# mit-han-lab/distrifuser

Hardware: NVIDIA H100
Metric: SDXL 50-step latency (ms/image) (lower is better)
Workload: dtype f16

## Files before the change

### distrifuser_b200/csrc/linear.cu

```cuda
#include <math.h>
#include <string.h>

#include "tc_ptx.cuh"

using namespace df;
using namespace df::tc;

namespace {

constexpr int BM = 128;
constexpr int BK = 64;
constexpr int NTHREADS = 288;
constexpr int NCONSUMER_WARPS = 8;
constexpr uint32_t A_BYTES = BM * BK * 2;

template <int BN> struct Stages { static constexpr int value = BN == 256 ? 4 : 5; };

template <int BN>
struct __align__(1024) SmemT {
  __half a[Stages<BN>::value][BM * BK];
  __half b[Stages<BN>::value][BN * BK];
  uint64_t full[Stages<BN>::value], empty[Stages<BN>::value];
};

enum { EPI_PLAIN = 0, EPI_GEGLU = 1 };

struct LinearArgs {
  const __half* bias;
  const __half* residual;
  __half* out;
  int64_t M;
  int N, K;
  int64_t ldr, ldo;
  int tiles_m, tiles_n;
  int publish;
  int pub_col0, pub_cols;
  int idx;
  uint32_t peer_mask;
  uint64_t tensor_off, slot_bytes;
  df_comm_t comm;
};

__device__ __forceinline__ float gelu_erf(float x) {
  const float z = fabsf(x) * 0.70710678118654752f;
  const float t = __fdividef(1.f, fmaf(0.3275911f, z, 1.f));
  float p = fmaf(1.061405429f, t, -1.453152027f);
  p = fmaf(p, t, 1.421413741f);
  p = fmaf(p, t, -0.284496736f);
  p = fmaf(p, t, 0.254829592f);
  const float e = p * t * __expf(-z * z);
  const float phi = x >= 0.f ? 1.f - 0.5f * e : 0.5f * e;
  return x * phi;
}

__device__ __forceinline__ float2 ld_h2f(const __half* p) { return __half22float2(*reinterpret_cast<const __half2*>(p)); }

template <int BN>
__device__ __forceinline__ void wgmma_tile(float* acc, uint64_t a_desc, uint64_t b_desc, uint32_t accumulate) {
  if constexpr (BN == 256) wgmma_ss_n256(acc, a_desc, b_desc, accumulate);
  else wgmma_ss_n160(acc, a_desc, b_desc, accumulate);
}

template <int EPI, int BN>
__global__ void __launch_bounds__(NTHREADS, 1)
linear_kernel(const __grid_constant__ CUtensorMap tm_a, const __grid_constant__ CUtensorMap tm_w, LinearArgs p) {
  static_assert(BN % 32 == 0 && BN <= 256 && (BN * BK * 2) % 1024 == 0, "tile shape");
  constexpr int STAGES = Stages<BN>::value;
  constexpr uint32_t B_BYTES = BN * BK * 2;
  using Smem = SmemT<BN>;
  extern __shared__ __align__(1024) uint8_t smem_raw[];
  Smem& sm = *reinterpret_cast<Smem*>(smem_raw);
  if ((smem_u32(smem_raw) & 1023u) != 0) __trap();
  const int warp = threadIdx.x >> 5, lane = threadIdx.x & 31;
  const int ntiles = p.tiles_m * p.tiles_n;
  const int kblocks = p.K / BK;

  if (threadIdx.x == 0) {
    for (int s = 0; s < STAGES; ++s) { mbar_init(&sm.full[s], 1); mbar_init(&sm.empty[s], NCONSUMER_WARPS); }
    asm volatile("fence.mbarrier_init.release.cluster;" ::: "memory");
  }
  __syncthreads();
  pdl_wait();

  if (warp == NCONSUMER_WARPS) {
    if (lane == 0) {
      prefetch_tmap(&tm_a);
      prefetch_tmap(&tm_w);
      uint32_t stage = 0, phase = 0;
      for (int tile = blockIdx.x; tile < ntiles; tile += gridDim.x) {
        const int tm = tile % p.tiles_m, tn = tile / p.tiles_m;
        for (int kb = 0; kb < kblocks; ++kb) {
          mbar_wait(&sm.empty[stage], phase ^ 1u);
          mbar_expect_tx(&sm.full[stage], A_BYTES + B_BYTES);
          tma_load_2d(sm.a[stage], &tm_a, &sm.full[stage], kb * BK, tm * BM);
          tma_load_2d(sm.b[stage], &tm_w, &sm.full[stage], kb * BK, tn * BN);
          if (++stage == STAGES) { stage = 0; phase ^= 1u; }
        }
      }
    }
  } else {
    const int wg = warp >> 2;
    const int c4 = lane & 3;
    const int rloc = wg * 64 + (warp & 3) * 16 + (lane >> 2);
    uint32_t pub_epoch = 0;
    if (p.publish) pub_epoch = p.comm.clock[0];
    uint32_t stage = 0, phase = 0;
    float acc[BN / 2];
    for (int tile = blockIdx.x; tile < ntiles; tile += gridDim.x) {
      const int tm = tile % p.tiles_m, tn = tile / p.tiles_m;
      fence_regs<BN / 2>(acc);
      uint32_t prev = 0;
      for (int kb = 0; kb < kblocks; ++kb) {
        mbar_wait(&sm.full[stage], phase);
        const uint32_t a_addr = smem_u32(sm.a[stage]) + wg * 64 * 128, b_addr = smem_u32(sm.b[stage]);
        wgmma_fence();
#pragma unroll
        for (int kk = 0; kk < BK / 16; ++kk)
          wgmma_tile<BN>(acc, smem_desc(a_addr + kk * 32, 16, 1024), smem_desc(b_addr + kk * 32, 16, 1024), (kb | kk) > 0);
        wgmma_commit();
        wgmma_wait<1>();
        if (kb > 0 && lane == 0) mbar_arrive(&sm.empty[prev]);
        prev = stage;
        if (++stage == STAGES) { stage = 0; phase ^= 1u; }
      }
      wgmma_wait<0>();
      fence_regs<BN / 2>(acc);
      if (lane == 0) mbar_arrive(&sm.empty[prev]);
#pragma unroll
      for (int h = 0; h < 2; ++h) {
        const int64_t grow = (int64_t)tm * BM + rloc + 8 * h;
        if (grow >= p.M) continue;
        if (EPI == EPI_GEGLU) {
          __half* dst = p.out + grow * p.ldo + tn * (BN / 2);
#pragma unroll
          for (int i = 0; i < BN / 16; ++i) {
            const int c = 8 * i + 2 * c4;
            float2 bh = make_float2(0.f, 0.f), bg = make_float2(0.f, 0.f);
            if (p.bias) { bh = ld_h2f(p.bias + tn * BN + c); bg = ld_h2f(p.bias + tn * BN + BN / 2 + c); }
            const float* hv = acc + 4 * i + 2 * h;
            const float* gv = acc + 4 * (i + BN / 16) + 2 * h;
            const float2 hf = __half22float2(__floats2half2_rn(hv[0] + bh.x, hv[1] + bh.y));
            const float2 gf = __half22float2(__floats2half2_rn(gv[0] + bg.x, gv[1] + bg.y));
            *reinterpret_cast<__half2*>(dst + c) = __floats2half2_rn(hf.x * gelu_erf(gf.x), hf.y * gelu_erf(gf.y));
          }
        } else {
          const int col0 = tn * BN;
          __half* dst = p.out + grow * p.ldo + col0;
          const __half* res = p.residual ? p.residual + grow * p.ldr + col0 : nullptr;
#pragma unroll
          for (int i = 0; i < BN / 8; ++i) {
            const int c = 8 * i + 2 * c4;
            const int col = col0 + c;
            if (col >= p.N) continue;
            float2 f = make_float2(acc[4 * i + 2 * h], acc[4 * i + 2 * h + 1]);
            if (p.bias) { const float2 bb = ld_h2f(p.bias + col); f.x += bb.x; f.y += bb.y; }
            __half2 o = __floats2half2_rn(f.x, f.y);
            if (res) o = __hadd2(o, *reinterpret_cast<const __half2*>(res + c));
            *reinterpret_cast<__half2*>(dst + c) = o;
            if (p.publish && col >= p.pub_col0) {
              const uint64_t off = slot_offset(p.comm, pub_epoch, p.tensor_off, p.slot_bytes, p.comm.rank) +
                                   ((uint64_t)grow * p.pub_cols + (col - p.pub_col0)) * 2;
              for (int q = 0; q < p.comm.world; ++q)
                if (p.peer_mask >> q & 1) *reinterpret_cast<__half2*>((char*)p.comm.base[q] + off) = o;
            }
          }
        }
      }
    }
  }
  if (p.publish) signal_when_last(p.comm, &p.comm.tickets[p.idx], gridDim.x, p.idx, p.peer_mask, p.comm.clock[0]);
}

int make_map2d(CUtensorMap* m, const void* base, int64_t rows, int K, int64_t pitch, int box_rows) {
  EncodeTiledFn enc = tensor_map_encoder();
  DF_REQUIRE(enc != nullptr, "cuTensorMapEncodeTiled is not available from this driver");
  cuuint64_t dims[2] = {(cuuint64_t)K, (cuuint64_t)rows};
  cuuint64_t strides[1] = {(cuuint64_t)pitch * 2};
  cuuint32_t box[2] = {BK, (cuuint32_t)box_rows};
  cuuint32_t estr[2] = {1, 1};
  CUresult r = enc(m, CU_TENSOR_MAP_DATA_TYPE_FLOAT16, 2, const_cast<void*>(base), dims, strides, box, estr,
                   CU_TENSOR_MAP_INTERLEAVE_NONE, CU_TENSOR_MAP_SWIZZLE_128B, CU_TENSOR_MAP_L2_PROMOTION_L2_256B,
                   CU_TENSOR_MAP_FLOAT_OOB_FILL_NONE);
  DF_REQUIRE(r == CUDA_SUCCESS, "cuTensorMapEncodeTiled failed (%d): base=%p rows=%lld K=%d pitch=%lld", (int)r, base,
             (long long)rows, K, (long long)pitch);
  return 0;
}

template <int EPI, int BN>
int launch_linear(const CUtensorMap& ta, const CUtensorMap& tw, const LinearArgs& args, int ctas, cudaStream_t st) {
  static bool attr_set = false;
  if (!attr_set) {
    DF_CHECK_CUDA(cudaFuncSetAttribute(linear_kernel<EPI, BN>, cudaFuncAttributeMaxDynamicSharedMemorySize, (int)sizeof(SmemT<BN>)));
    attr_set = true;
  }
  DF_CHECK_CUDA(launch_pdl(PDL_GEMM, linear_kernel<EPI, BN>, dim3(ctas), dim3(NTHREADS), sizeof(SmemT<BN>), st, ta, tw, args));
  return 0;
}

double tile_cost(int64_t M, int N, int bn, int ctas_avail) {
  const long long tm = (M + BM - 1) / BM, tn = (N + bn - 1) / bn, tiles = tm * tn;
  const long long rounds = (tiles + ctas_avail - 1) / ctas_avail;
  return (double)rounds * (bn + 64);
}

}

namespace {
int pick_bn(int64_t M, int N, int epilogue, int cap) {
  const bool ok160 = epilogue == EPI_PLAIN || N % 160 == 0, ok256 = epilogue == EPI_PLAIN || N % 256 == 0;
  if (!ok256) return ok160 ? 160 : 0;
  if (ok160 && tile_cost(M, N, 160, cap) < 0.97 * tile_cost(M, N, 256, cap)) return 160;
  return 256;
}
}

extern "C" int df_linear_supported(int64_t M, int N, int K, int epilogue) {
  if (M < 1 || N < 8 || N % 8 != 0 || K < BK || K % BK != 0) return 0;
  if (epilogue == EPI_GEGLU && pick_bn(M, N, epilogue, sm_count()) == 0) return 0;
  return 1;
}

extern "C" int df_linear_geglu_block(int64_t M, int N, int K) {
  (void)K;
  const int bn = pick_bn(M, N, EPI_GEGLU, sm_count());
  return bn / 2;
}

extern "C" int df_linear_fwd(df_comm_t comm, const void* a, const void* w, const void* bias, const void* residual, void* out,
                             int64_t M, int N, int K, int64_t lda, int64_t ldw, int64_t ldr, int64_t ldo, int epilogue,
                             int geglu_block, int publish, int pub_col0, int idx, uint32_t peer_mask, uint64_t tensor_off,
                             uint64_t slot_bytes, int max_ctas, void* stream) {
  DF_REQUIRE(epilogue == EPI_PLAIN || epilogue == EPI_GEGLU, "df_linear_fwd: unknown epilogue %d", epilogue);
  DF_REQUIRE(df_linear_supported(M, N, K, epilogue), "df_linear_fwd: unsupported shape M=%lld N=%d K=%d (N %% 8, K %% 64%s)",
             (long long)M, N, K, epilogue == EPI_GEGLU ? ", GEGLU: N % 256" : "");
  DF_REQUIRE(((uintptr_t)a % 16) == 0 && ((uintptr_t)w % 16) == 0 && ((uintptr_t)out % 16) == 0 && ((uintptr_t)bias % 16) == 0 &&
                 ((uintptr_t)residual % 16) == 0 && lda % 8 == 0 && ldw % 8 == 0 && ldo % 8 == 0 && ldr % 8 == 0,
             "df_linear_fwd: operands must be 16-byte aligned with pitches multiple of 8");
  DF_REQUIRE(!(publish && epilogue != EPI_PLAIN), "df_linear_fwd: publication is a plain-epilogue feature");
  LinearArgs args;
  memset(&args, 0, sizeof(args));
  args.bias = (const __half*)bias; args.residual = (const __half*)residual; args.out = (__half*)out;
  args.M = M; args.N = N; args.K = K; args.ldr = ldr; args.ldo = ldo;
  const int sms = sm_count();
  const int cap = max_ctas > 0 ? max_ctas : sms;
  int bn = pick_bn(M, N, epilogue, epilogue == EPI_GEGLU ? sms : cap);
  if (epilogue == EPI_GEGLU && geglu_block > 0) {
    DF_REQUIRE(geglu_block == 80 || geglu_block == 128, "df_linear_fwd: geglu_block must be 80 or 128");
    bn = 2 * geglu_block;
    DF_REQUIRE(N % bn == 0, "df_linear_fwd: interleave block %d does not tile N=%d", geglu_block, N);
  }
  args.tiles_m = (int)((M + BM - 1) / BM);
  args.tiles_n = (N + bn - 1) / bn;
  args.publish = publish && peer_mask != 0;
  args.comm = comm;
  if (args.publish) {
    DF_REQUIRE(pub_col0 >= 0 && pub_col0 < N && pub_col0 % 8 == 0, "df_linear_fwd: bad pub_col0");
    args.pub_col0 = pub_col0; args.pub_cols = N - pub_col0; args.idx = idx; args.peer_mask = peer_mask;
    args.tensor_off = tensor_off; args.slot_bytes = slot_bytes;
    DF_REQUIRE((uint64_t)M * args.pub_cols * 2 <= slot_bytes, "df_linear_fwd: published columns larger than the slot");
  }
  int ctas = args.tiles_m * args.tiles_n;
  if (ctas > cap) ctas = cap;
  if (ctas < 1) ctas = 1;
  CUtensorMap ta, tw;
  if (int rc = make_map2d(&ta, a, M, K, lda, BM)) return rc;
  if (int rc = make_map2d(&tw, w, N, K, ldw, bn)) return rc;
  cudaStream_t st = (cudaStream_t)stream;
  if (epilogue == EPI_GEGLU) {
    if (bn == 160) return launch_linear<EPI_GEGLU, 160>(ta, tw, args, ctas, st);
    return launch_linear<EPI_GEGLU, 256>(ta, tw, args, ctas, st);
  }
  if (bn == 160) return launch_linear<EPI_PLAIN, 160>(ta, tw, args, ctas, st);
  return launch_linear<EPI_PLAIN, 256>(ta, tw, args, ctas, st);
}
```

### distrifuser_b200/csrc/tc_ptx.cuh

```cuda
#pragma once
#include <cuda.h>

#include "common.cuh"

namespace df {
namespace tc {

__device__ __forceinline__ uint32_t smem_u32(const void* p) { return (uint32_t)__cvta_generic_to_shared(p); }

__device__ __forceinline__ void mbar_init(uint64_t* bar, uint32_t count) {
  asm volatile("mbarrier.init.shared::cta.b64 [%0], %1;" ::"r"(smem_u32(bar)), "r"(count));
}
__device__ __forceinline__ void mbar_expect_tx(uint64_t* bar, uint32_t bytes) {
  asm volatile("mbarrier.arrive.expect_tx.shared::cta.b64 _, [%0], %1;" ::"r"(smem_u32(bar)), "r"(bytes) : "memory");
}
__device__ __forceinline__ void mbar_arrive(uint32_t bar_addr) {
  asm volatile("mbarrier.arrive.shared::cta.b64 _, [%0];" ::"r"(bar_addr) : "memory");
}
__device__ __forceinline__ void mbar_arrive(uint64_t* bar) { mbar_arrive(smem_u32(bar)); }
#ifndef DF_TRYWAIT_HINT_NS
#define DF_TRYWAIT_HINT_NS 200000u
#endif
__device__ __forceinline__ bool mbar_try(uint32_t bar_addr, uint32_t parity) {
  uint32_t ok;
  asm volatile(
      "{\n\t.reg .pred p;\n\t"
      "mbarrier.try_wait.parity.shared::cta.b64 p, [%1], %2, %3;\n\t"
      "selp.u32 %0, 1, 0, p;\n\t}"
      : "=r"(ok)
      : "r"(bar_addr), "r"(parity), "r"(DF_TRYWAIT_HINT_NS)
      : "memory");
  return ok != 0;
}
__device__ __forceinline__ bool mbar_try(uint64_t* bar, uint32_t parity) { return mbar_try(smem_u32(bar), parity); }
__device__ __forceinline__ void mbar_wait(uint32_t bar, uint32_t parity) {
  if (mbar_try(bar, parity)) return;
  uint32_t polls = 0;
  uint64_t t0 = 0;
  while (!mbar_try(bar, parity)) {
    if ((++polls & 0x3FFu) == 0) {
      const uint64_t now = globaltimer_ns();
      if (t0 == 0) t0 = now;
      else if (now - t0 > 10000000000ull) {
#ifdef DF_MBAR_DEBUG
        printf("distrifuser_b200: mbarrier timeout (block %d,%d,%d thread %d bar@%u parity %u)\n", blockIdx.x, blockIdx.y, blockIdx.z,
               threadIdx.x, bar, parity);
#endif
        __trap();
      }
    }
  }
}

__device__ __forceinline__ void mbar_wait(uint64_t* bar, uint32_t parity) { mbar_wait(smem_u32(bar), parity); }

__device__ __forceinline__ void tma_load_4d(void* dst, const void* tmap, uint64_t* bar, int c0, int c1, int c2, int c3) {
  asm volatile(
      "cp.async.bulk.tensor.4d.shared::cluster.global.mbarrier::complete_tx::bytes [%0], [%1, {%3, %4, %5, %6}], [%2];"
      ::"r"(smem_u32(dst)), "l"((uint64_t)tmap), "r"(smem_u32(bar)), "r"(c0), "r"(c1), "r"(c2), "r"(c3)
      : "memory");
}
__device__ __forceinline__ void tma_load_2d(void* dst, const void* tmap, uint64_t* bar, int c0, int c1) {
  asm volatile(
      "cp.async.bulk.tensor.2d.shared::cluster.global.mbarrier::complete_tx::bytes [%0], [%1, {%3, %4}], [%2];"
      ::"r"(smem_u32(dst)), "l"((uint64_t)tmap), "r"(smem_u32(bar)), "r"(c0), "r"(c1)
      : "memory");
}
__device__ __forceinline__ void prefetch_tmap(const void* tmap) {
  asm volatile("prefetch.tensormap [%0];" ::"l"((uint64_t)tmap) : "memory");
}

__device__ __forceinline__ uint64_t smem_desc(uint32_t addr, uint32_t lbo_bytes, uint32_t sbo_bytes) {
  return (uint64_t)((addr & 0x3FFFFu) >> 4) | ((uint64_t)((lbo_bytes >> 4) & 0x3FFFu) << 16) |
         ((uint64_t)((sbo_bytes >> 4) & 0x3FFFu) << 32) | (1ull << 62);
}
__device__ __forceinline__ void wgmma_fence() { asm volatile("wgmma.fence.sync.aligned;" ::: "memory"); }
__device__ __forceinline__ void wgmma_commit() { asm volatile("wgmma.commit_group.sync.aligned;" ::: "memory"); }
template <int N>
__device__ __forceinline__ void wgmma_wait() { asm volatile("wgmma.wait_group.sync.aligned %0;" ::"n"(N) : "memory"); }
template <int N>
__device__ __forceinline__ void setmaxnreg_dec() { asm volatile("setmaxnreg.dec.sync.aligned.u32 %0;" ::"n"(N)); }
template <int N>
__device__ __forceinline__ void setmaxnreg_inc() { asm volatile("setmaxnreg.inc.sync.aligned.u32 %0;" ::"n"(N)); }
template <int ID, int COUNT>
__device__ __forceinline__ void named_bar_sync() { asm volatile("bar.sync %0, %1;" ::"n"(ID), "n"(COUNT) : "memory"); }
template <int ID, int COUNT>
__device__ __forceinline__ void named_bar_arrive() { asm volatile("bar.arrive %0, %1;" ::"n"(ID), "n"(COUNT) : "memory"); }
template <int N>
__device__ __forceinline__ void fence_regs(float* d) {
#pragma unroll
  for (int i = 0; i < N; ++i) asm volatile("" : "+f"(d[i])::"memory");
}

__device__ __forceinline__ void wgmma_ss_n64(float* d, uint64_t a_desc, uint64_t b_desc, uint32_t accumulate) {
  asm volatile(
      "{\n\t.reg .pred p;\n\tsetp.ne.b32 p, %34, 0;\n\t"
      "wgmma.mma_async.sync.aligned.m64n64k16.f32.f16.f16 {%0, %1, %2, %3, %4, %5, %6, %7, %8, %9, %10, %11, %12, %13, %14, %15, %16, %17, %18, %19, %20, %21, %22, %23, %24, %25, %26, %27, %28, %29, %30, %31}, %32, %33, p, 1, 1, 0, 0;\n\t}"
      : "+f"(d[0]), "+f"(d[1]), "+f"(d[2]), "+f"(d[3]), "+f"(d[4]), "+f"(d[5]), "+f"(d[6]), "+f"(d[7]), "+f"(d[8]), "+f"(d[9]), "+f"(d[10]), "+f"(d[11]), "+f"(d[12]), "+f"(d[13]), "+f"(d[14]), "+f"(d[15]), "+f"(d[16]), "+f"(d[17]), "+f"(d[18]), "+f"(d[19]), "+f"(d[20]), "+f"(d[21]), "+f"(d[22]), "+f"(d[23]), "+f"(d[24]), "+f"(d[25]), "+f"(d[26]), "+f"(d[27]), "+f"(d[28]), "+f"(d[29]), "+f"(d[30]), "+f"(d[31])
      : "l"(a_desc), "l"(b_desc), "r"(accumulate));
}
__device__ __forceinline__ void wgmma_ss_n128(float* d, uint64_t a_desc, uint64_t b_desc, uint32_t accumulate) {
  asm volatile(
      "{\n\t.reg .pred p;\n\tsetp.ne.b32 p, %66, 0;\n\t"
      "wgmma.mma_async.sync.aligned.m64n128k16.f32.f16.f16 {%0, %1, %2, %3, %4, %5, %6, %7, %8, %9, %10, %11, %12, %13, %14, %15, %16, %17, %18, %19, %20, %21, %22, %23, %24, %25, %26, %27, %28, %29, %30, %31, %32, %33, %34, %35, %36, %37, %38, %39, %40, %41, %42, %43, %44, %45, %46, %47, %48, %49, %50, %51, %52, %53, %54, %55, %56, %57, %58, %59, %60, %61, %62, %63}, %64, %65, p, 1, 1, 0, 0;\n\t}"
      : "+f"(d[0]), "+f"(d[1]), "+f"(d[2]), "+f"(d[3]), "+f"(d[4]), "+f"(d[5]), "+f"(d[6]), "+f"(d[7]), "+f"(d[8]), "+f"(d[9]), "+f"(d[10]), "+f"(d[11]), "+f"(d[12]), "+f"(d[13]), "+f"(d[14]), "+f"(d[15]), "+f"(d[16]), "+f"(d[17]), "+f"(d[18]), "+f"(d[19]), "+f"(d[20]), "+f"(d[21]), "+f"(d[22]), "+f"(d[23]), "+f"(d[24]), "+f"(d[25]), "+f"(d[26]), "+f"(d[27]), "+f"(d[28]), "+f"(d[29]), "+f"(d[30]), "+f"(d[31]), "+f"(d[32]), "+f"(d[33]), "+f"(d[34]), "+f"(d[35]), "+f"(d[36]), "+f"(d[37]), "+f"(d[38]), "+f"(d[39]), "+f"(d[40]), "+f"(d[41]), "+f"(d[42]), "+f"(d[43]), "+f"(d[44]), "+f"(d[45]), "+f"(d[46]), "+f"(d[47]), "+f"(d[48]), "+f"(d[49]), "+f"(d[50]), "+f"(d[51]), "+f"(d[52]), "+f"(d[53]), "+f"(d[54]), "+f"(d[55]), "+f"(d[56]), "+f"(d[57]), "+f"(d[58]), "+f"(d[59]), "+f"(d[60]), "+f"(d[61]), "+f"(d[62]), "+f"(d[63])
      : "l"(a_desc), "l"(b_desc), "r"(accumulate));
}

__device__ __forceinline__ void wgmma_ss_n160(float* d, uint64_t a_desc, uint64_t b_desc, uint32_t accumulate) {
  asm volatile(
      "{\n\t.reg .pred p;\n\tsetp.ne.b32 p, %82, 0;\n\t"
      "wgmma.mma_async.sync.aligned.m64n160k16.f32.f16.f16 {%0, %1, %2, %3, %4, %5, %6, %7, %8, %9, %10, %11, %12, %13, %14, %15, %16, %17, %18, %19, %20, %21, %22, %23, %24, %25, %26, %27, %28, %29, %30, %31, %32, %33, %34, %35, %36, %37, %38, %39, %40, %41, %42, %43, %44, %45, %46, %47, %48, %49, %50, %51, %52, %53, %54, %55, %56, %57, %58, %59, %60, %61, %62, %63, %64, %65, %66, %67, %68, %69, %70, %71, %72, %73, %74, %75, %76, %77, %78, %79}, %80, %81, p, 1, 1, 0, 0;\n\t}"
      : "+f"(d[0]), "+f"(d[1]), "+f"(d[2]), "+f"(d[3]), "+f"(d[4]), "+f"(d[5]), "+f"(d[6]), "+f"(d[7]), "+f"(d[8]), "+f"(d[9]), "+f"(d[10]), "+f"(d[11]), "+f"(d[12]), "+f"(d[13]), "+f"(d[14]), "+f"(d[15]), "+f"(d[16]), "+f"(d[17]), "+f"(d[18]), "+f"(d[19]), "+f"(d[20]), "+f"(d[21]), "+f"(d[22]), "+f"(d[23]), "+f"(d[24]), "+f"(d[25]), "+f"(d[26]), "+f"(d[27]), "+f"(d[28]), "+f"(d[29]), "+f"(d[30]), "+f"(d[31]), "+f"(d[32]), "+f"(d[33]), "+f"(d[34]), "+f"(d[35]), "+f"(d[36]), "+f"(d[37]), "+f"(d[38]), "+f"(d[39]), "+f"(d[40]), "+f"(d[41]), "+f"(d[42]), "+f"(d[43]), "+f"(d[44]), "+f"(d[45]), "+f"(d[46]), "+f"(d[47]), "+f"(d[48]), "+f"(d[49]), "+f"(d[50]), "+f"(d[51]), "+f"(d[52]), "+f"(d[53]), "+f"(d[54]), "+f"(d[55]), "+f"(d[56]), "+f"(d[57]), "+f"(d[58]), "+f"(d[59]), "+f"(d[60]), "+f"(d[61]), "+f"(d[62]), "+f"(d[63]), "+f"(d[64]), "+f"(d[65]), "+f"(d[66]), "+f"(d[67]), "+f"(d[68]), "+f"(d[69]), "+f"(d[70]), "+f"(d[71]), "+f"(d[72]), "+f"(d[73]), "+f"(d[74]), "+f"(d[75]), "+f"(d[76]), "+f"(d[77]), "+f"(d[78]), "+f"(d[79])
      : "l"(a_desc), "l"(b_desc), "r"(accumulate));
}

__device__ __forceinline__ void wgmma_ss_n256(float* d, uint64_t a_desc, uint64_t b_desc, uint32_t accumulate) {
  asm volatile(
      "{\n\t.reg .pred p;\n\tsetp.ne.b32 p, %130, 0;\n\t"
      "wgmma.mma_async.sync.aligned.m64n256k16.f32.f16.f16 {%0, %1, %2, %3, %4, %5, %6, %7, %8, %9, %10, %11, %12, %13, %14, %15, %16, %17, %18, %19, %20, %21, %22, %23, %24, %25, %26, %27, %28, %29, %30, %31, %32, %33, %34, %35, %36, %37, %38, %39, %40, %41, %42, %43, %44, %45, %46, %47, %48, %49, %50, %51, %52, %53, %54, %55, %56, %57, %58, %59, %60, %61, %62, %63, %64, %65, %66, %67, %68, %69, %70, %71, %72, %73, %74, %75, %76, %77, %78, %79, %80, %81, %82, %83, %84, %85, %86, %87, %88, %89, %90, %91, %92, %93, %94, %95, %96, %97, %98, %99, %100, %101, %102, %103, %104, %105, %106, %107, %108, %109, %110, %111, %112, %113, %114, %115, %116, %117, %118, %119, %120, %121, %122, %123, %124, %125, %126, %127}, %128, %129, p, 1, 1, 0, 0;\n\t}"
      : "+f"(d[0]), "+f"(d[1]), "+f"(d[2]), "+f"(d[3]), "+f"(d[4]), "+f"(d[5]), "+f"(d[6]), "+f"(d[7]), "+f"(d[8]), "+f"(d[9]), "+f"(d[10]), "+f"(d[11]), "+f"(d[12]), "+f"(d[13]), "+f"(d[14]), "+f"(d[15]), "+f"(d[16]), "+f"(d[17]), "+f"(d[18]), "+f"(d[19]), "+f"(d[20]), "+f"(d[21]), "+f"(d[22]), "+f"(d[23]), "+f"(d[24]), "+f"(d[25]), "+f"(d[26]), "+f"(d[27]), "+f"(d[28]), "+f"(d[29]), "+f"(d[30]), "+f"(d[31]), "+f"(d[32]), "+f"(d[33]), "+f"(d[34]), "+f"(d[35]), "+f"(d[36]), "+f"(d[37]), "+f"(d[38]), "+f"(d[39]), "+f"(d[40]), "+f"(d[41]), "+f"(d[42]), "+f"(d[43]), "+f"(d[44]), "+f"(d[45]), "+f"(d[46]), "+f"(d[47]), "+f"(d[48]), "+f"(d[49]), "+f"(d[50]), "+f"(d[51]), "+f"(d[52]), "+f"(d[53]), "+f"(d[54]), "+f"(d[55]), "+f"(d[56]), "+f"(d[57]), "+f"(d[58]), "+f"(d[59]), "+f"(d[60]), "+f"(d[61]), "+f"(d[62]), "+f"(d[63]), "+f"(d[64]), "+f"(d[65]), "+f"(d[66]), "+f"(d[67]), "+f"(d[68]), "+f"(d[69]), "+f"(d[70]), "+f"(d[71]), "+f"(d[72]), "+f"(d[73]), "+f"(d[74]), "+f"(d[75]), "+f"(d[76]), "+f"(d[77]), "+f"(d[78]), "+f"(d[79]), "+f"(d[80]), "+f"(d[81]), "+f"(d[82]), "+f"(d[83]), "+f"(d[84]), "+f"(d[85]), "+f"(d[86]), "+f"(d[87]), "+f"(d[88]), "+f"(d[89]), "+f"(d[90]), "+f"(d[91]), "+f"(d[92]), "+f"(d[93]), "+f"(d[94]), "+f"(d[95]), "+f"(d[96]), "+f"(d[97]), "+f"(d[98]), "+f"(d[99]), "+f"(d[100]), "+f"(d[101]), "+f"(d[102]), "+f"(d[103]), "+f"(d[104]), "+f"(d[105]), "+f"(d[106]), "+f"(d[107]), "+f"(d[108]), "+f"(d[109]), "+f"(d[110]), "+f"(d[111]), "+f"(d[112]), "+f"(d[113]), "+f"(d[114]), "+f"(d[115]), "+f"(d[116]), "+f"(d[117]), "+f"(d[118]), "+f"(d[119]), "+f"(d[120]), "+f"(d[121]), "+f"(d[122]), "+f"(d[123]), "+f"(d[124]), "+f"(d[125]), "+f"(d[126]), "+f"(d[127])
      : "l"(a_desc), "l"(b_desc), "r"(accumulate));
}

__device__ __forceinline__ void wgmma_rs_n64(float* d, const uint32_t* a, uint64_t b_desc, uint32_t accumulate) {
  asm volatile(
      "{\n\t.reg .pred p;\n\tsetp.ne.b32 p, %37, 0;\n\t"
      "wgmma.mma_async.sync.aligned.m64n64k16.f32.f16.f16 {%0, %1, %2, %3, %4, %5, %6, %7, %8, %9, %10, %11, %12, %13, %14, %15, %16, %17, %18, %19, %20, %21, %22, %23, %24, %25, %26, %27, %28, %29, %30, %31}, {%32, %33, %34, %35}, %36, p, 1, 1, 1;\n\t}"
      : "+f"(d[0]), "+f"(d[1]), "+f"(d[2]), "+f"(d[3]), "+f"(d[4]), "+f"(d[5]), "+f"(d[6]), "+f"(d[7]), "+f"(d[8]), "+f"(d[9]), "+f"(d[10]), "+f"(d[11]), "+f"(d[12]), "+f"(d[13]), "+f"(d[14]), "+f"(d[15]), "+f"(d[16]), "+f"(d[17]), "+f"(d[18]), "+f"(d[19]), "+f"(d[20]), "+f"(d[21]), "+f"(d[22]), "+f"(d[23]), "+f"(d[24]), "+f"(d[25]), "+f"(d[26]), "+f"(d[27]), "+f"(d[28]), "+f"(d[29]), "+f"(d[30]), "+f"(d[31])
      : "r"(a[0]), "r"(a[1]), "r"(a[2]), "r"(a[3]), "l"(b_desc), "r"(accumulate));
}


__device__ __forceinline__ float ex2(float x) {
  float y;
  asm("ex2.approx.ftz.f32 %0, %1;" : "=f"(y) : "f"(x));
  return y;
}
__device__ __forceinline__ float ex2_poly(float x) {
  x = fmaxf(x, -127.f);
  const float r = __fadd_rd(x, 12582912.f);
  const float f = x - (r - 12582912.f);
  float q = fmaf(f, 0.077119089663028717041015625f, 0.227564394474029541015625f);
  q = fmaf(q, f, 0.695146143436431884765625f);
  q = fmaf(q, f, 1.f);
  return __int_as_float(__float_as_int(q) + (__float_as_int(r) << 23));
}
__device__ __forceinline__ uint32_t pack_h2(float lo, float hi) {
  __half2 h = __floats2half2_rn(lo, hi);
  return *reinterpret_cast<uint32_t*>(&h);
}


}
}
```

Measured before the change: 1566.

## Stage GEGLU epilogue in swizzled shared memory and write out via TMA store

The GEGLU epilogue of the linear kernel now writes its fp16 outputs into a per-warpgroup swizzled shared-memory staging buffer instead of issuing scattered half2 global stores. One thread per warpgroup then issues 2D TMA bulk stores, with a separate output tensor map built at launch. The goal is fully coalesced, asynchronous output writes that overlap the next tile's mainloop. In exchange it uses extra shared memory (which may pressure stage counts), adds named-barrier syncs and proxy fences, and encodes a tensor map on the host at every launch.

```diff
diff --git a/distrifuser_b200/csrc/linear.cu b/distrifuser_b200/csrc/linear.cu
--- a/distrifuser_b200/csrc/linear.cu
+++ b/distrifuser_b200/csrc/linear.cu
@@ -16,14 +16,27 @@
 
 template <int BN> struct Stages { static constexpr int value = BN == 256 ? 4 : 5; };
 
-template <int BN>
+enum { EPI_PLAIN = 0, EPI_GEGLU = 1 };
+
+template <int BN> struct StoreBox {
+  static constexpr int cols = (BN / 2) % 64 == 0 ? 64 : 16;
+  static constexpr int row_bytes = cols * 2;
+};
+
+template <int EPI, int BN>
 struct __align__(1024) SmemT {
   __half a[Stages<BN>::value][BM * BK];
   __half b[Stages<BN>::value][BN * BK];
+  __half c[EPI == EPI_GEGLU ? BM * BN / 2 : 8];
   uint64_t full[Stages<BN>::value], empty[Stages<BN>::value];
 };
 
-enum { EPI_PLAIN = 0, EPI_GEGLU = 1 };
+template <int BN>
+__device__ __forceinline__ uint32_t staging_offset(int r, int c) {
+  constexpr int SW = StoreBox<BN>::cols, RB = StoreBox<BN>::row_bytes;
+  const uint32_t o = (uint32_t)((c / SW) * 64 * RB + r * RB + (c % SW) * 2);
+  return o ^ (((o >> 7) & (RB / 16 - 1)) << 4);
+}
 
 struct LinearArgs {
   const __half* bias;
@@ -63,11 +76,12 @@
 
 template <int EPI, int BN>
 __global__ void __launch_bounds__(NTHREADS, 1)
-linear_kernel(const __grid_constant__ CUtensorMap tm_a, const __grid_constant__ CUtensorMap tm_w, LinearArgs p) {
+linear_kernel(const __grid_constant__ CUtensorMap tm_a, const __grid_constant__ CUtensorMap tm_w,
+              const __grid_constant__ CUtensorMap tm_o, LinearArgs p) {
   static_assert(BN % 32 == 0 && BN <= 256 && (BN * BK * 2) % 1024 == 0, "tile shape");
   constexpr int STAGES = Stages<BN>::value;
   constexpr uint32_t B_BYTES = BN * BK * 2;
-  using Smem = SmemT<BN>;
+  using Smem = SmemT<EPI, BN>;
   extern __shared__ __align__(1024) uint8_t smem_raw[];
   Smem& sm = *reinterpret_cast<Smem*>(smem_raw);
   if ((smem_u32(smem_raw) & 1023u) != 0) __trap();
@@ -102,6 +116,8 @@
     const int wg = warp >> 2;
     const int c4 = lane & 3;
     const int rloc = wg * 64 + (warp & 3) * 16 + (lane >> 2);
+    const bool store_issuer = (threadIdx.x & 127) == 0;
+    uint8_t* staging = reinterpret_cast<uint8_t*>(sm.c) + wg * (64 * BN);
     uint32_t pub_epoch = 0;
     if (p.publish) pub_epoch = p.comm.clock[0];
     uint32_t stage = 0, phase = 0;
@@ -126,12 +142,12 @@
       wgmma_wait<0>();
       fence_regs<BN / 2>(acc);
       if (lane == 0) mbar_arrive(&sm.empty[prev]);
-#pragma unroll
-      for (int h = 0; h < 2; ++h) {
-        const int64_t grow = (int64_t)tm * BM + rloc + 8 * h;
-        if (grow >= p.M) continue;
-        if (EPI == EPI_GEGLU) {
-          __half* dst = p.out + grow * p.ldo + tn * (BN / 2);
+      if constexpr (EPI == EPI_GEGLU) {
+        if (store_issuer) bulk_wait_read_all();
+        named_bar_sync(1 + wg, 128);
+#pragma unroll
+        for (int h = 0; h < 2; ++h) {
+          const int r = rloc - wg * 64 + 8 * h;
 #pragma unroll
           for (int i = 0; i < BN / 16; ++i) {
             const int c = 8 * i + 2 * c4;
@@ -141,9 +157,24 @@
             const float* gv = acc + 4 * (i + BN / 16) + 2 * h;
             const float2 hf = __half22float2(__floats2half2_rn(hv[0] + bh.x, hv[1] + bh.y));
             const float2 gf = __half22float2(__floats2half2_rn(gv[0] + bg.x, gv[1] + bg.y));
-            *reinterpret_cast<__half2*>(dst + c) = __floats2half2_rn(hf.x * gelu_erf(gf.x), hf.y * gelu_erf(gf.y));
+            *reinterpret_cast<__half2*>(staging + staging_offset<BN>(r, c)) =
+                __floats2half2_rn(hf.x * gelu_erf(gf.x), hf.y * gelu_erf(gf.y));
           }
-        } else {
+        }
+        fence_proxy_async_smem();
+        named_bar_sync(1 + wg, 128);
+        if (store_issuer) {
+          constexpr int SW = StoreBox<BN>::cols;
+#pragma unroll
+          for (int b = 0; b < BN / 2 / SW; ++b)
+            tma_store_2d(&tm_o, staging + b * 64 * StoreBox<BN>::row_bytes, tn * (BN / 2) + b * SW, tm * BM + wg * 64);
+          bulk_commit();
+        }
+      } else {
+#pragma unroll
+        for (int h = 0; h < 2; ++h) {
+          const int64_t grow = (int64_t)tm * BM + rloc + 8 * h;
+          if (grow >= p.M) continue;
           const int col0 = tn * BN;
           __half* dst = p.out + grow * p.ldo + col0;
           const __half* res = p.residual ? p.residual + grow * p.ldr + col0 : nullptr;
@@ -167,33 +198,44 @@
         }
       }
     }
+    if (EPI == EPI_GEGLU && store_issuer) bulk_wait_all();
   }
   if (p.publish) signal_when_last(p.comm, &p.comm.tickets[p.idx], gridDim.x, p.idx, p.peer_mask, p.comm.clock[0]);
 }
 
-int make_map2d(CUtensorMap* m, const void* base, int64_t rows, int K, int64_t pitch, int box_rows) {
+int make_map2d(CUtensorMap* m, const void* base, int64_t rows, int cols, int64_t pitch, int box_cols, int box_rows,
+               CUtensorMapSwizzle swizzle) {
   EncodeTiledFn enc = tensor_map_encoder();
   DF_REQUIRE(enc != nullptr, "cuTensorMapEncodeTiled is not available from this driver");
-  cuuint64_t dims[2] = {(cuuint64_t)K, (cuuint64_t)rows};
+  cuuint64_t dims[2] = {(cuuint64_t)cols, (cuuint64_t)rows};
   cuuint64_t strides[1] = {(cuuint64_t)pitch * 2};
-  cuuint32_t box[2] = {BK, (cuuint32_t)box_rows};
+  cuuint32_t box[2] = {(cuuint32_t)box_cols, (cuuint32_t)box_rows};
   cuuint32_t estr[2] = {1, 1};
   CUresult r = enc(m, CU_TENSOR_MAP_DATA_TYPE_FLOAT16, 2, const_cast<void*>(base), dims, strides, box, estr,
-                   CU_TENSOR_MAP_INTERLEAVE_NONE, CU_TENSOR_MAP_SWIZZLE_128B, CU_TENSOR_MAP_L2_PROMOTION_L2_256B,
+                   CU_TENSOR_MAP_INTERLEAVE_NONE, swizzle, CU_TENSOR_MAP_L2_PROMOTION_L2_256B,
                    CU_TENSOR_MAP_FLOAT_OOB_FILL_NONE);
-  DF_REQUIRE(r == CUDA_SUCCESS, "cuTensorMapEncodeTiled failed (%d): base=%p rows=%lld K=%d pitch=%lld", (int)r, base,
-             (long long)rows, K, (long long)pitch);
+  DF_REQUIRE(r == CUDA_SUCCESS, "cuTensorMapEncodeTiled failed (%d): base=%p rows=%lld cols=%d pitch=%lld", (int)r, base,
+             (long long)rows, cols, (long long)pitch);
   return 0;
 }
 
 template <int EPI, int BN>
 int launch_linear(const CUtensorMap& ta, const CUtensorMap& tw, const LinearArgs& args, int ctas, cudaStream_t st) {
+  constexpr size_t smem = sizeof(SmemT<EPI, BN>);
   static bool attr_set = false;
   if (!attr_set) {
-    DF_CHECK_CUDA(cudaFuncSetAttribute(linear_kernel<EPI, BN>, cudaFuncAttributeMaxDynamicSharedMemorySize, (int)sizeof(SmemT<BN>)));
+    DF_CHECK_CUDA(cudaFuncSetAttribute(linear_kernel<EPI, BN>, cudaFuncAttributeMaxDynamicSharedMemorySize, (int)smem));
     attr_set = true;
   }
-  DF_CHECK_CUDA(launch_pdl(PDL_GEMM, linear_kernel<EPI, BN>, dim3(ctas), dim3(NTHREADS), sizeof(SmemT<BN>), st, ta, tw, args));
+  CUtensorMap to;
+  memset(&to, 0, sizeof(to));
+  if (EPI == EPI_GEGLU) {
+    constexpr int SW = StoreBox<BN>::cols;
+    if (int rc = make_map2d(&to, args.out, args.M, args.N / 2, args.ldo, SW, 64,
+                            SW == 64 ? CU_TENSOR_MAP_SWIZZLE_128B : CU_TENSOR_MAP_SWIZZLE_32B))
+      return rc;
+  }
+  DF_CHECK_CUDA(launch_pdl(PDL_GEMM, linear_kernel<EPI, BN>, dim3(ctas), dim3(NTHREADS), smem, st, ta, tw, to, args));
   return 0;
 }
 
@@ -263,8 +305,8 @@
   if (ctas > cap) ctas = cap;
   if (ctas < 1) ctas = 1;
   CUtensorMap ta, tw;
-  if (int rc = make_map2d(&ta, a, M, K, lda, BM)) return rc;
-  if (int rc = make_map2d(&tw, w, N, K, ldw, bn)) return rc;
+  if (int rc = make_map2d(&ta, a, M, K, lda, BK, BM, CU_TENSOR_MAP_SWIZZLE_128B)) return rc;
+  if (int rc = make_map2d(&tw, w, N, K, ldw, BK, bn, CU_TENSOR_MAP_SWIZZLE_128B)) return rc;
   cudaStream_t st = (cudaStream_t)stream;
   if (epilogue == EPI_GEGLU) {
     if (bn == 160) return launch_linear<EPI_GEGLU, 160>(ta, tw, args, ctas, st);
diff --git a/distrifuser_b200/csrc/tc_ptx.cuh b/distrifuser_b200/csrc/tc_ptx.cuh
--- a/distrifuser_b200/csrc/tc_ptx.cuh
+++ b/distrifuser_b200/csrc/tc_ptx.cuh
@@ -66,6 +66,14 @@
       ::"r"(smem_u32(dst)), "l"((uint64_t)tmap), "r"(smem_u32(bar)), "r"(c0), "r"(c1)
       : "memory");
 }
+__device__ __forceinline__ void tma_store_2d(const void* tmap, const void* src, int c0, int c1) {
+  asm volatile("cp.async.bulk.tensor.2d.global.shared::cta.bulk_group [%0, {%2, %3}], [%1];"
+               ::"l"((uint64_t)tmap), "r"(smem_u32(src)), "r"(c0), "r"(c1) : "memory");
+}
+__device__ __forceinline__ void bulk_commit() { asm volatile("cp.async.bulk.commit_group;" ::: "memory"); }
+__device__ __forceinline__ void bulk_wait_read_all() { asm volatile("cp.async.bulk.wait_group.read 0;" ::: "memory"); }
+__device__ __forceinline__ void bulk_wait_all() { asm volatile("cp.async.bulk.wait_group 0;" ::: "memory"); }
+__device__ __forceinline__ void fence_proxy_async_smem() { asm volatile("fence.proxy.async.shared::cta;" ::: "memory"); }
 __device__ __forceinline__ void prefetch_tmap(const void* tmap) {
   asm volatile("prefetch.tensormap [%0];" ::"l"((uint64_t)tmap) : "memory");
 }
@@ -84,6 +92,9 @@
 __device__ __forceinline__ void setmaxnreg_inc() { asm volatile("setmaxnreg.inc.sync.aligned.u32 %0;" ::"n"(N)); }
 template <int ID, int COUNT>
 __device__ __forceinline__ void named_bar_sync() { asm volatile("bar.sync %0, %1;" ::"n"(ID), "n"(COUNT) : "memory"); }
+__device__ __forceinline__ void named_bar_sync(uint32_t id, uint32_t count) {
+  asm volatile("bar.sync %0, %1;" ::"r"(id), "r"(count) : "memory");
+}
 template <int ID, int COUNT>
 __device__ __forceinline__ void named_bar_arrive() { asm volatile("bar.arrive %0, %1;" ::"n"(ID), "n"(COUNT) : "memory"); }
 template <int N>
```

After: 1538 (median of 6 runs). About the same (-1.8%).
